# HansiZeng/scaling-retriever

Measured on AMD Instinct MI355X. Metric: MSMARCO-Dev queries/sec end-to-end (query encode + dense brute-force top-1000), higher is better.
Workload: dtype f32

## Files before the change

### include/sr_hip.h

```cpp
#ifndef SR_HIP_H
#define SR_HIP_H
#include <stdint.h>
#ifdef __cplusplus
extern "C" {
#endif

#define SR_OK 0
#define SR_ERR_INVALID 1
#define SR_ERR_HIP 2
#define SR_ERR_NOMEM 3
#define SR_ERR_UNSUPPORTED 4

#define SR_DTYPE_F32 0
#define SR_DTYPE_BF16 1
#define SR_DTYPE_F16 2

typedef void* sr_stream;

const char* sr_last_error(void);
int sr_version(void);
int sr_max_topk(void);

typedef struct sr_dense_index sr_dense_index;

// ... 250 lines not shown
                       const float* d_rope_cos, const float* d_rope_sin, int32_t n_rope, int32_t head_dim,
                       const float* d_bias, const int32_t* d_seq_of, const float* d_out_scale, int32_t out_nseg,
                       sr_stream stream);
int sr_gemm_qkv_rope(const void* d_A, const void* d_W, int32_t M, int32_t N, int32_t K, void* d_C,
                     const int32_t* d_pos, const float* d_rope_cos, const float* d_rope_sin,
                     int32_t n_rope, int32_t head_dim, sr_stream stream);
int sr_gemm_qkv_rope_bias(const void* d_A, const void* d_W, int32_t M, int32_t N, int32_t K, void* d_C,
                          const int32_t* d_pos, const float* d_rope_cos, const float* d_rope_sin,
                          int32_t n_rope, int32_t head_dim, const float* d_bias, int32_t fp32_out, sr_stream stream);
int sr_attention_varlen(const void* d_qkv, void* d_out, const int32_t* d_cu_seqlens, const int32_t* d_pos,
                        const uint8_t* d_key_valid, const float* d_rope_cos, const float* d_rope_sin,
                        int32_t B, int32_t num_heads, int32_t num_kv_heads, int32_t head_dim, sr_stream stream);
int sr_attention_varlen_f32(const float* d_qkv, float* d_out_f32, void* d_out_planes, int32_t fp32_planes,
                            const int32_t* d_cu_seqlens, const uint8_t* d_key_valid, int32_t B, int32_t num_heads,
                            int32_t num_kv_heads, int32_t head_dim, int32_t max_seqlen, sr_stream stream);
int sr_rmsnorm_bf16(float* d_x, const float* d_embed, const int32_t* d_tok_id, const void* d_delta, const float* d_norm_w,
                    void* d_xn, float* d_xn_f32, float eps, int32_t T, int32_t H, sr_stream stream);
int sr_dense_head_pool(const float* d_x, const float* d_norm_w, const int32_t* d_cu_seqlens, const int32_t* d_pos,
                       const int32_t* d_pool_start, float eps, int32_t B, int32_t T, int32_t H, void* d_stats, float* d_out,
                       sr_stream stream);
int sr_sparse_finish(float* d_out, int64_t n, float scale, int32_t round_bf16, sr_stream stream);
int sr_encode_plan(const int64_t* d_input_ids, const int64_t* d_attention_mask, int32_t B, int32_t L, int32_t mode, int32_t vocab,
                   const int32_t* d_row_shift, int32_t* d_span_start, int32_t* d_span_len, int32_t* d_pool_start,
                   int32_t* d_row_len, int32_t* d_cu_seqlens, int32_t* d_tok_id, int32_t* d_pos, uint8_t* d_key_valid,
                   int32_t* d_seq_of, int64_t capacity, int64_t* n_tokens, sr_stream stream);
int sr_split_bf16(const float* d_src, int64_t n, void* d_p0, void* d_p1, void* d_p2, sr_stream stream);
int sr_topk_replay(const float* d_scores, const int64_t* d_ids, int64_t nq, int64_t n_stream, const int64_t* h_steps, int n_steps,
                   int k, int k2, int64_t select_over, int filter, int seg_n, int seg_group, float tau2_init, float pad_score,
                   float* d_out_scores, int64_t* d_out_ids, int32_t* d_out_counts, float* d_trace_tau, float* d_trace_tau2,
                   int32_t* d_trace_cand, int32_t* d_trace_run, uint64_t* d_trace_keys, sr_stream stream);
// ... 22 lines not shown
```

### scaling_retriever_amd/_lib.py

```python
import contextlib
import ctypes
import os
import threading

_HERE = os.path.dirname(os.path.abspath(__file__))
LIB_PATH = os.environ.get("SR_HIP_LIB") or os.path.join(_HERE, "libsr_hip.so")

SR_OK, SR_ERR_INVALID, SR_ERR_HIP, SR_ERR_NOMEM, SR_ERR_UNSUPPORTED = 0, 1, 2, 3, 4
SR_DTYPE_F32, SR_DTYPE_BF16, SR_DTYPE_F16 = 0, 1, 2
SR_FUSE_RRF, SR_FUSE_MINMAX = 0, 1

c_void_p, c_int, c_int32, c_int64, c_float, c_char_p = (ctypes.c_void_p, ctypes.c_int, ctypes.c_int32,
                                                         ctypes.c_int64, ctypes.c_float, ctypes.c_char_p)


class SrModelConfig(ctypes.Structure):
    _fields_ = [
        ("vocab_size", c_int32), ("hidden_size", c_int32), ("intermediate_size", c_int32), ("num_layers", c_int32),
        ("num_heads", c_int32), ("num_kv_heads", c_int32), ("head_dim", c_int32),
        ("rms_norm_eps", c_float), ("rope_theta", c_float), ("rope_llama3", c_int32),
        ("rope_factor", c_float), ("rope_low_freq_factor", c_float), ("rope_high_freq_factor", c_float),
        ("rope_original_max_pos", c_int32), ("tie_word_embeddings", c_int32), ("has_lm_head", c_int32),
        ("max_batch_tokens", c_int32), ("max_batch_seqs", c_int32), ("fp32_planes", c_int32),
        ("attention_bias", c_int32),
# ... 135 lines not shown
    "sr_rmsnorm_bf16": (c_int, [c_void_p, c_void_p, c_void_p, c_void_p, c_void_p, c_void_p, c_void_p, c_float, c_int32, c_int32, c_void_p]),
    "sr_dense_head_pool": (c_int, [c_void_p, c_void_p, c_void_p, c_void_p, c_void_p, c_float, c_int32, c_int32, c_int32, c_void_p, c_void_p,
                                   c_void_p]),
    "sr_sparse_finish": (c_int, [c_void_p, c_int64, c_float, c_int32, c_void_p]),
    "sr_encode_plan": (c_int, [c_void_p, c_void_p, c_int32, c_int32, c_int32, c_int32, c_void_p, c_void_p, c_void_p, c_void_p, c_void_p,
                               c_void_p, c_void_p, c_void_p, c_void_p, c_void_p, c_int64, ctypes.POINTER(c_int64), c_void_p]),
    "sr_split_bf16": (c_int, [c_void_p, c_int64, c_void_p, c_void_p, c_void_p, c_void_p]),
    "sr_gemm_qkv_rope": (c_int, [c_void_p, c_void_p, c_int32, c_int32, c_int32, c_void_p, c_void_p, c_void_p, c_void_p,
                                 c_int32, c_int32, c_void_p]),
    "sr_gemm_qkv_rope_bias": (c_int, [c_void_p, c_void_p, c_int32, c_int32, c_int32, c_void_p, c_void_p, c_void_p, c_void_p,
                                      c_int32, c_int32, c_void_p, c_int32, c_void_p]),
    "sr_attention_varlen": (c_int, [c_void_p, c_void_p, c_void_p, c_void_p, c_void_p, c_void_p, c_void_p, c_int32,
                                    c_int32, c_int32, c_int32, c_void_p]),
    "sr_attention_varlen_f32": (c_int, [c_void_p, c_void_p, c_void_p, c_int32, c_void_p, c_void_p, c_int32, c_int32, c_int32,
                                        c_int32, c_int32, c_void_p]),
    "sr_sparse_compact": (c_int, [c_void_p, c_int64, c_int64, c_void_p, c_void_p, c_void_p, c_int64,
                                  ctypes.POINTER(c_int64), c_void_p]),
    "sr_sparse_compact_topm": (c_int, [c_void_p, c_int64, c_int64, c_int64, c_void_p, c_void_p, c_void_p, c_int64,
                                       ctypes.POINTER(c_int64), c_void_p]),
}

_lib = None
_lock = threading.Lock()


class SrHipError(RuntimeError):
    pass


def _bind(path):
    if not os.path.exists(path):
        raise SrHipError(
            f"{path} not found: the HIP extension is not built. There is no CPU fallback; "
            "run `make -C scaling_retriever_amd/csrc` (needs hipcc, targets gfx950).")
    import torch
    lib = ctypes.CDLL(path)
    for name, (res, args) in SIGNATURES.items():
        fn = getattr(lib, name)
        fn.restype = res
        fn.argtypes = args
    return lib


def load():
    global _lib
    with _lock:
        if _lib is None:
            _lib = _bind(LIB_PATH)
        return _lib


@contextlib.contextmanager
def library(path):
    global _lib
    other = _bind(os.path.abspath(path))
    with _lock:
        keep, _lib = _lib, other
    try:
        yield other
    finally:
        with _lock:
            _lib = keep


def check(rc, what=""):
    if rc == SR_OK:
        return
    msg = load().sr_last_error().decode("utf-8", "replace")
    if rc == SR_ERR_INVALID:
        raise ValueError(f"{what}: {msg}" if what else msg)
# ... 16 lines not shown
```

### scaling_retriever_amd/csrc/api.hip

```cpp
#include "kernels.h"
#include <stdlib.h>
#include <string>
#include <vector>

static thread_local std::string g_last_error;

void sr_set_error(const char* fmt, ...) {
    char buf[1024];
    va_list ap;
    va_start(ap, fmt);
    vsnprintf(buf, sizeof(buf), fmt, ap);
    va_end(ap);
    g_last_error = buf;
}

int sr_cu_count() {
    static int per_dev[SR_MAX_DEVICES] = {};
    int d = 0;
    if (hipGetDevice(&d) != hipSuccess || d < 0 || d >= SR_MAX_DEVICES) d = 0;
    if (per_dev[d] == 0) {
        int n = 0;
        if (hipDeviceGetAttribute(&n, hipDeviceAttributeMultiprocessorCount, d) != hipSuccess || n <= 0) { (void)hipGetLastError(); n = 256; }
        per_dev[d] = n;
    }
// ... 65 lines not shown
extern "C" int sr_attention_varlen_f32(const float* d_qkv, float* d_out_f32, void* d_out_planes, int32_t fp32_planes,
                                       const int32_t* d_cu_seqlens, const uint8_t* d_key_valid, int32_t B, int32_t num_heads,
                                       int32_t num_kv_heads, int32_t head_dim, int32_t max_seqlen, sr_stream stream) {
    SR_REQUIRE(d_qkv && d_cu_seqlens && d_key_valid, "sr_attention_varlen_f32: null pointer");
    SR_REQUIRE((d_out_f32 != nullptr) != (d_out_planes != nullptr), "sr_attention_varlen_f32: pass exactly one of d_out_f32 / d_out_planes");
    SR_REQUIRE(d_out_f32 || fp32_planes == 2 || fp32_planes == 3, "sr_attention_varlen_f32: fp32_planes %d (2 or 3 for plane output)", fp32_planes);
    SR_REQUIRE(B >= 0 && max_seqlen >= 0 && num_heads > 0 && num_kv_heads > 0 && head_dim > 0, "sr_attention_varlen_f32: bad sizes");
    SR_REQUIRE((uintptr_t)d_qkv % 16 == 0 && (uintptr_t)d_out_f32 % 16 == 0 && (uintptr_t)d_out_planes % 8 == 0,
               "sr_attention_varlen_f32: d_qkv and d_out_f32 must be 16-byte aligned, d_out_planes 8-byte aligned");
    AttnF32Args a{};
    a.qkv = d_qkv; a.out_f32 = d_out_f32; a.out = (bf16_t*)d_out_planes; a.cu_seqlens = d_cu_seqlens; a.key_valid = d_key_valid;
    a.B = B; a.nh = num_heads; a.nkv = num_kv_heads; a.hd = head_dim;
    a.scale = 1.0f / sqrtf((float)head_dim); a.max_seqlen = max_seqlen;
    if (!d_out_f32) a.out_map = split_map_a(fp32_planes);
    return launch_attention_f32(a, (hipStream_t)stream);
}

extern "C" int sr_gemm_f16_scaled(const void* d_A, const void* d_W, int32_t M, int32_t N, int32_t K, const float* d_a_scale,
                                  const float* d_w_scale, float* d_C, sr_stream stream) {
    SR_REQUIRE(d_A && d_W && d_C && d_a_scale && d_w_scale, "sr_gemm_f16_scaled: null pointer");
    GemmArgs g{};
    g.A = (const bf16_t*)d_A; g.W = (const bf16_t*)d_W; g.M = M; g.N = N; g.K = K; g.C = d_C; g.a_scale = d_a_scale; g.w_scale = d_w_scale;
    return launch_gemm_bf16(EPI_RESID_F32_H, g, (hipStream_t)stream);
}

extern "C" int sr_rows_split_f16(float* d_src, const float* d_embed, const int32_t* d_tok_id, const float* d_norm_w, float eps,
                                 int32_t T, int32_t K, int32_t nseg, void* d_planes, float* d_a_inv, const float* d_gu_cmax,
                                 float* d_act_sc, float* d_act_inv, sr_stream stream) {
    SR_REQUIRE(d_src && d_planes && d_a_inv, "sr_rows_split_f16: null pointer");
    SR_REQUIRE((d_embed == nullptr) == (d_tok_id == nullptr), "sr_rows_split_f16: pass both d_embed and d_tok_id or neither");
// ... 103 lines not shown
```

### scaling_retriever_amd/csrc/attention_f32.hip

```cpp
#include "kernels.h"
#include <math.h>

#define AF_KC 64
#define AF_RPW 4
#define AF_ROWS 16

__device__ inline float af_mul_rn(float a, float b) {
#pragma clang fp contract(off)
    return a * b;
}

template <int HD>
__global__ __launch_bounds__(256) void attention_f32_kernel(AttnF32Args a) {
    constexpr int DPL = HD / 64;
    __shared__ float Ks[AF_KC][HD + 1];
    __shared__ float qs[AF_ROWS][HD];
    __shared__ float ps[AF_ROWS][AF_KC];
    __shared__ unsigned char kval[AF_KC];
    const int b = blockIdx.x, h = blockIdx.y;
    const int tid = threadIdx.x, lane = tid & 63, wave = tid >> 6;
    const int t0 = a.cu_seqlens[b];
    const int S = a.cu_seqlens[b + 1] - t0;
    const int r0 = blockIdx.z * AF_ROWS;
    if (r0 >= S || S <= a.only_gt) return;
// ... 210 lines not shown
    const float s0 = af_quad_xor(hi1 ? x0 : x1, 0xB1), s1 = af_quad_xor(hi1 ? x2 : x3, 0xB1);
    if (hi1) { x0 = s0; x2 = s1; } else { x1 = s0; x3 = s1; }
    x = f32x4{x0, x1, x2, x3};
}

__host__ __device__ constexpr int af_mfma_waves(int hd, int nkb) {
    return nkb == 0 ? 1 : (hd == 64 ? (nkb == 1 ? 8 : 6) : (nkb <= 2 ? 5 : 4));
}

template <int HD, int NKB>
__global__ __launch_bounds__(256, af_mfma_waves(HD, NKB)) void attention_f32_mfma_kernel(AttnF32Args a) {
    constexpr int LDK = HD + 1, CB = HD / 16;
    constexpr bool OLD = NKB == 0;
    constexpr int MKB = OLD ? 4 : NKB;
    extern __shared__ float af_smem[];
    const int b = blockIdx.x, kvh = blockIdx.y;
    const int tid = threadIdx.x, lane = tid & 63, wave = tid >> 6;
    const int t0 = a.cu_seqlens[b];
    const int S = a.cu_seqlens[b + 1] - t0;
    if (S <= 0 || S > a.only_le) return;
    const int nkb = (S + 15) >> 4;
    if (!OLD && (a.nkb_only ? nkb != a.nkb_only : nkb > NKB)) return;
    const int SP = nkb * 16;
    float* Ks = af_smem;
    float* Vs = Ks + SP * LDK;
    const int G = a.nh / a.nkv;
    const int h = kvh * G + wave;
    const int ld = (a.nh + 2 * a.nkv) * HD;
    const int koff = a.nh * HD + kvh * HD, voff = (a.nh + a.nkv) * HD + kvh * HD;
    const int g = lane >> 4, c = lane & 15;
    f32x4 qv[CB];
    auto load_q = [&](int qb) {
#pragma unroll
        for (int i = 0; i < CB; ++i) {
// ... 161 lines not shown
                    bf16_t* orow = a.out + (int64_t)(t0 + row) * ldo;
                    for (int sg = 0; sg < a.out_map.n_seg; ++sg) {
                        const int pl = a.out_map.plane[sg];
                        bf16x4 w;
#pragma unroll
                        for (int e = 0; e < 4; ++e) w[e] = (short)(pl == 0 ? p[e][0] : (pl == 1 ? p[e][1] : p[e][2]));
                        *reinterpret_cast<bf16x4*>(orow + (int64_t)sg * a.nh * HD + col) = w;
                    }
                }
            }
        }
    }
}

template <int HD, int NKB>
static int launch_attention_f32_mfma_cfg(const AttnF32Args& a, size_t lds, hipStream_t s) {
    static DeviceOnce attr_once;
    if (bool* slot = attr_once.pending()) {
        constexpr int max_sp = NKB ? 16 * NKB : 64;
        SR_CHECK_HIP(hipFuncSetAttribute(reinterpret_cast<const void*>(&attention_f32_mfma_kernel<HD, NKB>),
                                         hipFuncAttributeMaxDynamicSharedMemorySize, (int)(sizeof(float) * (2 * max_sp + (NKB ? 0 : 64)) * (HD + 1))));
        *slot = true;
    }
    const dim3 grid((unsigned)a.B, (unsigned)a.nkv), block(256);
    SR_REQUIRE(grid.y <= 65535, "attention(fp32): grid too large");
    hipLaunchKernelGGL((attention_f32_mfma_kernel<HD, NKB>), grid, block, lds, s, a);
    SR_CHECK_LAUNCH();
    return SR_OK;
}

template <int HD>
static int launch_attention_f32_mfma_class(const AttnF32Args& a, int nkb, hipStream_t s) {
    const size_t lds = sizeof(float) * (size_t)(2 * 16 * nkb) * (HD + 1);
    switch (nkb) {
        case 1: return launch_attention_f32_mfma_cfg<HD, 1>(a, lds, s);
        case 2: return launch_attention_f32_mfma_cfg<HD, 2>(a, lds, s);
        case 3: return launch_attention_f32_mfma_cfg<HD, 3>(a, lds, s);
        default: return launch_attention_f32_mfma_cfg<HD, 4>(a, lds, s);
    }
}

template <int HD>
static int launch_attention_f32_mfma(const AttnF32Args& a_in, hipStream_t s) {
    AttnF32Args a = a_in;
    const int top = (int)ceil_div64(a.max_seqlen < 64 ? a.max_seqlen : 64, 16);
    const char* env = sr_dev_getenv("SR_ATTN_F32_LAYOUT");
    if (env && *env == '0') {
        const size_t lds = sizeof(float) * (size_t)(2 * 16 * top + 4 * 16) * (HD + 1);
        return launch_attention_f32_mfma_cfg<HD, 0>(a, lds, s);
    }
    const bool force = env && *env == '2';
    if (!a.have_classes && !force) {
        a.nkb_only = 0;
        return launch_attention_f32_mfma_class<HD>(a, top, s);
    }
    for (int nkb = 1; nkb <= top; ++nkb) {
        if (a.have_classes && a.class_seqs[nkb - 1] == 0) continue;
        a.nkb_only = nkb;
        SR_TRY(launch_attention_f32_mfma_class<HD>(a, nkb, s));
    }
    return SR_OK;
}

int launch_attention_f32(const AttnF32Args& a_in, hipStream_t s) {
    AttnF32Args a = a_in;
    SR_REQUIRE(a.nh % a.nkv == 0, "attention(fp32): num_heads %d not a multiple of num_kv_heads %d", a.nh, a.nkv);
    SR_REQUIRE(a.out_f32 || (a.out_map.n_seg >= 1 && a.out_map.n_seg <= SR_MAX_SEG), "attention(fp32): bad segment map");
    if (a.B == 0 || a.max_seqlen <= 0) return SR_OK;
    const int G = a.nh / a.nkv;
    a.only_le = 0; a.only_gt = 0;
    const char* env_m = sr_dev_getenv("SR_ATTN_F32_MFMA");
    if (G == 4 && (a.hd == 64 || a.hd == 128) && !(env_m && *env_m == '0')) {
        a.only_le = 64;
        SR_TRY(a.hd == 64 ? launch_attention_f32_mfma<64>(a, s) : launch_attention_f32_mfma<128>(a, s));
// ... 26 lines not shown
```

### scaling_retriever_amd/csrc/encoder.hip

```cpp
#include "encoder_model.h"
#include <math.h>

struct Pass {
    sr_model* m;
    hipStream_t s;
    int B, T;
    int max_len;
    int attn_class[4];
    bool fused_on, fused_all;
};

static int ensure_fp32_workspace(sr_model* m) {
    if (m->xs) return SR_OK;
    const sr_model_config& c = m->cfg;
    SR_REQUIRE(c.fp32_planes > 0, "encode(fp32): the model was created with fp32_planes = 0 (bf16 regime only)");
    const int64_t Tm = m->Tm, nsg = split_map_a(c.fp32_planes).n_seg;
    const ModelDims& d = m->d;
    DeviceArena& mem = m->mem_fp32;
    auto allocate = [&]() -> int {
        SR_TRY(mem.alloc(m->xs, Tm * d.H * nsg, true));
        SR_TRY(mem.alloc(m->qkv_f, Tm * d.n_qkv, true));
        SR_TRY(mem.alloc(m->attn_s, Tm * d.nq * nsg, true));
        SR_TRY(mem.alloc(m->act_s, Tm * d.I * nsg, true));
        if (c.fp32_planes != SR_FP32_PLANES_F16) return SR_OK;
        SR_TRY(mem.alloc(m->attn_f, Tm * d.nq, true));
        SR_TRY(mem.alloc(m->act_f, Tm * d.I, true));
        SR_TRY(mem.alloc(m->xs_i, Tm, true));
        SR_TRY(mem.alloc(m->attn_i, Tm, true));
        SR_TRY(mem.alloc(m->act_i, Tm, true));
        SR_TRY(mem.alloc(m->act_sc, Tm, true));
        return SR_OK;
    };
    if (allocate() != SR_OK) {
        mem.release();
        sr_set_error("encode(fp32): hipMalloc of the fp32-regime workspace failed (%lld tokens)", (long long)Tm);
        return SR_ERR_NOMEM;
    }
    return SR_OK;
// ... 9 lines not shown
    g.a_nseg = nseg; g.a_scale = a_inv; g.w_scale = w_inv;
    return g;
}
static void set_rope(GemmArgs& g, const sr_model* m, const float* bias) {
    g.pos = m->pos; g.rope_cos = m->rope_cos; g.rope_sin = m->rope_sin; g.n_rope = m->d.nq + m->d.nkv; g.head_dim = m->d.hd;
    g.bias = bias;
}
static AttnF32Args attn_f32_args(const Pass& p) {
    const sr_model* m = p.m;
    AttnF32Args a{};
    a.qkv = m->qkv_f; a.cu_seqlens = m->cu; a.key_valid = m->key_valid;
    a.B = p.B; a.nh = m->cfg.num_heads; a.nkv = m->cfg.num_kv_heads; a.hd = m->d.hd;
    a.scale = 1.0f / sqrtf((float)m->d.hd); a.max_seqlen = p.max_len;
    a.have_classes = 1;
    for (int n = 0; n < 4; ++n) a.class_seqs[n] = p.attn_class[n];
    return a;
}
static int split_rows(const Pass& p, float* src, const float* w, bf16_t* dst, float* inv, int K, int nseg) {
    return launch_rows_split_f16(src, nullptr, nullptr, w, dst, inv, p.T, K, p.m->cfg.rms_norm_eps, nseg, nullptr, nullptr, nullptr, p.s);
}

static int layer_bf16(const Pass& p, int li) {
    sr_model* m = p.m;
    const ModelDims& d = m->d;
    const LayerW& l = m->layers[li];
    const float eps = m->cfg.rms_norm_eps;
    const int T = p.T;
    hipStream_t s = p.s;
    if (li == 0) SR_TRY(launch_rmsnorm(m->x, m->embed, m->tok_id, nullptr, l.ln1, m->xn, nullptr, T, d.H, eps, s));
    else SR_TRY(launch_rmsnorm(m->x, nullptr, nullptr, m->delta, l.ln1, m->xn, nullptr, T, d.H, eps, s));
// ... 54 lines not shown
    SR_TRY(launch_gemm_bf16(EPI_RESID_F32_H, gemm_f16(m->attn_s, m->attn_i, l.wo_s, l.wo_i, l.o_seg, T, d.H, d.nq, m->x), s));
    if (p.fused_on && (l.fused_act || p.fused_all)) {
        SR_TRY(launch_rows_split_f16(m->x, nullptr, nullptr, l.ln2, m->xs, m->xs_i, T, d.H, eps, l.gu_seg, m->gu_cmax + li, m->act_sc,
                                     m->act_i, s));
        g = gemm_f16(m->xs, m->xs_i, l.wgu_s, l.wgu_i, l.gu_seg, T, 2 * d.I, d.H, m->act_s);
        g.out_scale = m->act_sc; g.out_nseg = l.down_seg;
        SR_TRY(launch_gemm_bf16(EPI_SWIGLU_SPLIT_H, g, s));
    } else {
        SR_TRY(split_rows(p, m->x, l.ln2, m->xs, m->xs_i, d.H, l.gu_seg));
        SR_TRY(launch_gemm_bf16(EPI_SWIGLU_F32_H, gemm_f16(m->xs, m->xs_i, l.wgu_s, l.wgu_i, l.gu_seg, T, 2 * d.I, d.H, m->act_f), s));
        SR_TRY(split_rows(p, m->act_f, nullptr, m->act_s, m->act_i, d.I, l.down_seg));
    }
    return launch_gemm_bf16(EPI_RESID_F32_H, gemm_f16(m->act_s, m->act_i, l.wdown_s, l.wdown_i, l.down_seg, T, d.H, d.I, m->x), s);
}

static int plan_batch(sr_model* m, const int64_t* d_ids, const int64_t* d_mask, int B, int L, int mode, const int32_t* d_shift, Pass& p) {
    hipStream_t s = p.s;
    SR_TRY(launch_plan_rows(d_mask, B, L, mode, m->span_start, m->span_len, m->pool_start, m->row_len, d_shift, m->cu, s));
    SR_CHECK_HIP(hipMemcpyAsync(m->h_cu, m->cu, (size_t)(B + 1) * 4, hipMemcpyDeviceToHost, s));
    SR_CHECK_HIP(hipStreamSynchronize(s));
    p.B = B;
    p.T = m->h_cu[B];
    p.max_len = 0;
    for (int n = 0; n < 4; ++n) p.attn_class[n] = 0;
    for (int b = 0; b < B; ++b) {
        const int len = m->h_cu[b + 1] - m->h_cu[b];
        p.max_len = len > p.max_len ? len : p.max_len;
        if (len >= 1 && len <= 64) ++p.attn_class[(len - 1) >> 4];
    }
    SR_REQUIRE(p.T <= m->Tm, "encode: batch packs to %d tokens, workspace holds %d (raise max_batch_tokens or split the batch)", p.T, m->Tm);
    m->last_T = p.T;
    if (p.T == 0) return SR_OK;
    return launch_plan_tokens(d_ids, d_mask, B, L, m->span_start, m->cu, m->tok_id, m->pos, m->key_valid, m->seq_of, m->d.V, mode, d_shift, s);
}

static int model_forward(sr_model* m, const int64_t* d_ids, const int64_t* d_mask, int B, int L, int mode, int prec, const int32_t* d_shift,
                         Pass& p) {
    const sr_model_config& c = m->cfg;
    SR_REQUIRE(m->finalized, "encode: sr_model_finalize was not called");
    SR_REQUIRE(B >= 1 && L >= 1, "encode: bad batch shape [%d, %d]", B, L);
    SR_REQUIRE(B <= m->Bm, "encode: batch of %d sequences exceeds max_batch_seqs %d", B, m->Bm);
    SR_REQUIRE(L <= m->max_pos, "encode: sequence length %d exceeds %d", L, m->max_pos);
    SR_REQUIRE(d_ids && d_mask, "encode: null input");
    if (prec == PREC_FP32) SR_TRY(ensure_fp32_workspace(m));
    SR_TRY(plan_batch(m, d_ids, d_mask, B, L, mode, d_shift, p));
    if (p.T == 0) return SR_OK;
    const bool f16p = prec == PREC_FP32 && c.fp32_planes == SR_FP32_PLANES_F16;
    if (f16p) {
        const char* env_fa = sr_dev_getenv("SR_FP32_FUSED_ACT");
        p.fused_on = !(env_fa && *env_fa == '0');
        p.fused_all = env_fa && *env_fa == '1';
    }
    for (int li = 0; li < c.num_layers; ++li)
        SR_TRY(prec == PREC_BF16 ? layer_bf16(p, li) : (f16p ? layer_f16_planes(p, li) : layer_f32_planes(p, li)));
    if (prec == PREC_BF16)
        SR_TRY(launch_rmsnorm(m->x, nullptr, nullptr, m->delta, nullptr, nullptr, nullptr, p.T, m->d.H, c.rms_norm_eps, p.s));
    return SR_OK;
}

static int head_dense(const Pass& p, int prec, float* d_out) {
// ... 108 lines not shown
```

### scaling_retriever_amd/csrc/encoder_kernels.hip

```cpp
#include "kernels.h"
#include <math.h>

__global__ void plan_rows_kernel(const int64_t* __restrict__ mask, int B, int L, int mode, int* __restrict__ span_start,
                                 int* __restrict__ span_len, int* __restrict__ pool_start, int* __restrict__ row_len,
                                 const int* __restrict__ row_shift) {
    const int b = blockIdx.x;
    const int lane = threadIdx.x;
    int len = 0, first = L, last = -1;
    for (int p = lane; p < L; p += 64) {
        if (mask[(int64_t)b * L + p] != 0) {
            ++len;
            first = p < first ? p : first;
            last = p > last ? p : last;
        }
    }
    for (int off = 32; off > 0; off >>= 1) {
        len += __shfl_xor(len, off);
        const int f = __shfl_xor(first, off), l = __shfl_xor(last, off);
        first = f < first ? f : first;
        last = l > last ? l : last;
    }
    if (lane == 0) {
        int st, ln, ps;
        if (len == 0) {
// ... 19 lines not shown
    const int tid = threadIdx.x;
    const int per = (B + 255) / 256;
    const int b0 = tid * per, b1 = (b0 + per) < B ? (b0 + per) : B;
    int s = 0;
    for (int b = b0; b < b1; ++b) s += span_len[b];
    part[tid] = s;
    __syncthreads();
    if (tid == 0) {
        int run = 0;
        for (int i = 0; i < 256; ++i) { const int v = part[i]; part[i] = run; run += v; }
        cu[B] = run;
    }
    __syncthreads();
    int run = part[tid];
    for (int b = b0; b < b1; ++b) { cu[b] = run; run += span_len[b]; }
}

__global__ void plan_tokens_kernel(const int64_t* __restrict__ ids, const int64_t* __restrict__ mask, int L,
                                   const int* __restrict__ span_start, const int* __restrict__ cu, int* __restrict__ tok_id,
                                   int* __restrict__ pos, unsigned char* __restrict__ key_valid, int* __restrict__ seq_of,
                                   int vocab, int mode, const int* __restrict__ row_shift) {
    const int b = blockIdx.x;
    const int t0 = cu[b], n = cu[b + 1] - t0, st = span_start[b];
    const int shift = row_shift ? row_shift[b] : 0;
    for (int j = threadIdx.x; j < n; j += blockDim.x) {
        const int p = st + j;
        int64_t id = ids[(int64_t)b * L + p];
        id = id < 0 ? 0 : (id >= vocab ? vocab - 1 : id);
        tok_id[t0 + j] = (int)id;
        pos[t0 + j] = p - shift < 0 ? 0 : p - shift;
        const bool valid = mask[(int64_t)b * L + p] != 0;
        key_valid[t0 + j] = valid ? 1 : 0;
        seq_of[t0 + j] = (mode != 0 && !valid) ? -2 : b;
    }
}

int launch_plan_rows(const int64_t* mask, int B, int L, int mode, int* span_start, int* span_len, int* pool_start, int* row_len,
                     const int* row_shift, int* cu, hipStream_t s) {
    hipLaunchKernelGGL(plan_rows_kernel, dim3(B), dim3(64), 0, s, mask, B, L, mode, span_start, span_len, pool_start, row_len, row_shift);
    hipLaunchKernelGGL(plan_scan_kernel, dim3(1), dim3(256), 0, s, span_len, B, cu);
    SR_CHECK_LAUNCH();
    return SR_OK;
}
int launch_plan_tokens(const int64_t* ids, const int64_t* mask, int B, int L, const int* span_start, const int* cu, int* tok_id, int* pos,
                       unsigned char* key_valid, int* seq_of, int vocab, int mode, const int* row_shift, hipStream_t s) {
    hipLaunchKernelGGL(plan_tokens_kernel, dim3(B), dim3(128), 0, s, ids, mask, L, span_start, cu, tok_id, pos, key_valid, seq_of, vocab,
                       mode, row_shift);
    SR_CHECK_LAUNCH();
    return SR_OK;
}

template <int NCH>
__global__ __launch_bounds__(256) void rmsnorm_kernel(float* __restrict__ x, const float* __restrict__ embed,
                                                      const int* __restrict__ tok_id, const bf16_t* __restrict__ delta,
                                                      const float* __restrict__ w, bf16_t* __restrict__ xn,
                                                      float* __restrict__ xn_f32, int T, int H, float eps) {
    const int t = blockIdx.x * 4 + (threadIdx.x >> 6);
    const int lane = threadIdx.x & 63;
// ... 200 lines not shown
```

### scaling_retriever_amd/csrc/encoder_model.h

```cpp
#pragma once
#include "kernels.h"
#include <mutex>
#include <vector>

enum { PREC_BF16 = 0, PREC_FP32 = 1 };

struct ModelDims {
    int H, I, V;
    int nq, nkv;
    int n_qkv;
    int hd;
};

struct DeviceArena {
    struct Block { void* p; void** slot; };
    std::vector<Block> blocks;
    DeviceArena() = default;
    DeviceArena(const DeviceArena&) = delete;
    DeviceArena& operator=(const DeviceArena&) = delete;
    ~DeviceArena() { release(); }
    template <typename T>
    int alloc(T*& ptr, int64_t n, bool zero = false) {
        const size_t bytes = (size_t)n * sizeof(T);
        void* p = nullptr;
// ... 55 lines not shown
    bf16_t* xn = nullptr;
    bf16_t* qkv = nullptr;
    bf16_t* attn = nullptr;
    bf16_t* act = nullptr;
    bf16_t* delta = nullptr;
    int *span_start = nullptr, *span_len = nullptr, *pool_start = nullptr, *row_len = nullptr, *cu = nullptr;
    int *tok_id = nullptr, *pos = nullptr, *seq_of = nullptr;
    unsigned char* key_valid = nullptr;
    bf16_t* xs = nullptr;
    float* qkv_f = nullptr;
    bf16_t* attn_s = nullptr;
    bf16_t* act_s = nullptr;
    float *attn_f = nullptr, *act_f = nullptr;
    float *xs_i = nullptr, *attn_i = nullptr, *act_i = nullptr;
    float* act_sc = nullptr;
    DeviceArena mem;
    DeviceArena mem_fp32;
    int* h_cu = nullptr;
    int last_T = 0;
    std::mutex mu;
    StreamOrder order;

    sr_model() = default;
    sr_model(const sr_model&) = delete;
    ~sr_model() {
        if (h_cu) (void)hipHostFree(h_cu);
        order.release();
    }
};
```

### scaling_retriever_amd/csrc/gemm_bf16.hip

```cpp
#include "kernels.h"
#include <math.h>
#include <stdlib.h>
#include <string.h>
#include <type_traits>

typedef __bf16 mfma_bf16x8 __attribute__((ext_vector_type(8)));
typedef _Float16 mfma_f16x8 __attribute__((ext_vector_type(8)));
template <bool F16>
__device__ __forceinline__ f32x4 sr_mma(const mfma_bf16x8& w, const mfma_bf16x8& a, const f32x4& c) {
    if constexpr (F16)
        return __builtin_amdgcn_mfma_f32_16x16x32_f16(__builtin_bit_cast(mfma_f16x8, w), __builtin_bit_cast(mfma_f16x8, a), c, 0, 0, 0);
    else
        return __builtin_amdgcn_mfma_f32_16x16x32_bf16(w, a, c, 0, 0, 0);
}
__device__ __forceinline__ f32x4 sr_rope_lo(const f32x4& x1, const f32x4& x2, const f32x4& c, const f32x4& s) {
#pragma clang fp contract(off)
    f32x4 y;
#pragma unroll
    for (int r = 0; r < 4; ++r) { const float a = x1[r] * c[r], b = x2[r] * s[r]; y[r] = a - b; }
    return y;
}
__device__ __forceinline__ f32x4 sr_rope_hi(const f32x4& x1, const f32x4& x2, const f32x4& c, const f32x4& s) {
#pragma clang fp contract(off)
    f32x4 y;
// ... 672 lines not shown
                const int tok = it * 4 + (lane_e >> 4), pl = (lane_e >> 3) & 1, pc = lane_e & 7;
                const sr_i32x4 v = *reinterpret_cast<const sr_i32x4*>(stg + tok * 256 + pl * 128 + ((pc ^ (tok & 7)) << 4));
                const int m = mrow + tok, n = nb + pc * 8;
                if (m < g.M && n < half_n) {
                    bf16_t* crow = out_c + (int64_t)m * ldc + n;
                    if (pl == 0) {
                        *reinterpret_cast<sr_i32x4*>(crow) = v;
                    } else {
                        *reinterpret_cast<sr_i32x4*>(crow + half_n) = v;
                        if (seg3) *reinterpret_cast<sr_i32x4*>(crow + 2 * half_n) = v;
                    }
                }
            }
            __builtin_amdgcn_sched_barrier(0);
        }
    } else if constexpr (BEPI == EPI_STORE_BF16 || BEPI == EPI_STORE_F32 || BEPI == EPI_RESID_F32) {
#pragma unroll
        for (int j = 0; j < MB; ++j) {
            const int m = m0 + wm * MB * 16 + j * 16 + frow;
            if (m >= g.M) continue;
#pragma unroll
            for (int i = 0; i < NB; ++i) {
                const int n = n0 + wn * NB * 16 + i * 16 + fg * 4;
                if (n >= g.N) continue;
                const f32x4 v = acc[i][j];
                if constexpr (BEPI == EPI_STORE_BF16) {
                    bf16x4 o;
                    o[0] = (short)f32_to_bf16(v[0]);
                    o[1] = (short)f32_to_bf16(v[1]);
                    o[2] = (short)f32_to_bf16(v[2]);
                    o[3] = (short)f32_to_bf16(v[3]);
                    *reinterpret_cast<bf16x4*>(reinterpret_cast<bf16_t*>(g.C) + (int64_t)m * g.N + n) = o;
                } else if constexpr (BEPI == EPI_STORE_F32) {
                    *reinterpret_cast<f32x4*>(reinterpret_cast<float*>(g.C) + (int64_t)m * g.N + n) = v;
                } else {
                    f32x4* p = reinterpret_cast<f32x4*>(reinterpret_cast<float*>(g.C) + (int64_t)m * g.N + n);
                    f32x4 x = *p;
                    x += v;
                    *p = x;
                }
            }
        }
    } else if constexpr (E::QKV_ROPE) {
        constexpr bool F32OUT = E::OUT_BYTES == 4;
        const int hd = g.head_dim, hb = hd / 32;
        auto put = [&](int64_t off, const f32x4& v) {
            if constexpr (F32OUT) {
                *reinterpret_cast<f32x4*>(reinterpret_cast<float*>(g.C) + off) = v;
            } else {
                bf16x4 o;
#pragma unroll
                for (int r = 0; r < 4; ++r) o[r] = (short)f32_to_bf16(v[r]);
                *reinterpret_cast<bf16x4*>(reinterpret_cast<bf16_t*>(g.C) + off) = o;
            }
// ... 366 lines not shown
```

### scaling_retriever_amd/csrc/kernels.h

```cpp
#pragma once
#include "common.h"

typedef unsigned short bf16_t;

enum GemmEpilogue {
    EPI_STORE_BF16 = 0,
    EPI_RESID_F32 = 1,
    EPI_SWIGLU = 2,
    EPI_SEGMAX = 3,
    EPI_STORE_F32 = 4,
    EPI_QKV_ROPE = 5,
    EPI_QKV_ROPE_F32 = 6,
    EPI_SWIGLU_SPLIT = 7,
    EPI_SWIGLU_F32 = 8,
    EPI_H_FIRST = 9,
    EPI_QKV_ROPE_F32_H = 9, EPI_RESID_F32_H = 10, EPI_SWIGLU_F32_H = 11, EPI_SEGMAX_H = 12,
    EPI_SWIGLU_SPLIT_H = 13,
    EPI_SWIGLU_SPLITH_BASE = 14,
};

#define SR_MAX_SEG 6
struct SplitMap {
    int n_seg;
    int plane[SR_MAX_SEG];
// ... 35 lines not shown
int launch_gemm_bf16(GemmEpilogue epi, const GemmArgs& g, hipStream_t s);

int launch_rows_split_f16(float* x, const float* embed, const int* tok, const float* w, bf16_t* xs, float* inv, int T, int K, float eps,
                          int nseg, const float* gu_cmax, float* act_sc, float* act_inv, hipStream_t s);
int launch_gu_cmax(const bf16_t* wgu_s, const float* wgu_i, int I, int K, int nseg, float* cmax, hipStream_t s);
int launch_gu_pair_samples(const bf16_t* wgu_s, const float* wgu_i, int I, int K, int nseg, int ns, float* p, hipStream_t s);

int launch_rmsnorm_split(float* x, const float* embed, const int* tok_id, const float* w, bf16_t* xs, int T, int H, float eps,
                         const SplitMap& map, hipStream_t s);
int launch_rmsnorm(float* x, const float* embed, const int* tok_id, const bf16_t* delta, const float* w, bf16_t* xn, float* xn_f32, int T,
                   int H, float eps, hipStream_t s);
int launch_plan_rows(const int64_t* mask, int B, int L, int mode, int* span_start, int* span_len, int* pool_start, int* row_len,
                     const int* row_shift, int* cu, hipStream_t s);
int launch_plan_tokens(const int64_t* ids, const int64_t* mask, int B, int L, const int* span_start, const int* cu, int* tok_id, int* pos,
                       unsigned char* key_valid, int* seq_of, int vocab, int mode, const int* row_shift, hipStream_t s);
int launch_dense_head(const float* x, const float* w, float2* stats, const int* cu, const int* pos, const int* pool_start, float* out,
                      int B, int T, int H, float eps, hipStream_t s);
int launch_sparse_finish(float* out, int64_t n, float scale, int round_bf16, hipStream_t s);

struct AttnArgs {
    const bf16_t* qkv;
    bf16_t* out;
    const int* cu_seqlens;
    const int* pos;
    const unsigned char* key_valid;
    const float* rope_cos;
    const float* rope_sin;
    int B, nh, nkv, hd;
    float scale;
    int apply_rope;
// ... 2 lines not shown
int launch_attention(const AttnArgs& a, hipStream_t s);

struct AttnF32Args {
    const float* qkv;
    float* out_f32;
    bf16_t* out;
    const int* cu_seqlens;
    const unsigned char* key_valid;
    int B, nh, nkv, hd;
    float scale;
    int max_seqlen;
    SplitMap out_map;
    int only_le = 0, only_gt = 0;
    int have_classes = 0, class_seqs[4] = {0, 0, 0, 0};
    int nkb_only = 0;
};
int launch_attention_f32(const AttnF32Args& a, hipStream_t s);
```

Before: 16000.

## Compact attention grids per length class and batch residual epilogue loads

Adds a device planning kernel that buckets sequences by key-block count (length classes up to 64) and writes compact (start,len) spans, so each per-class fp32 attention launch covers only its own sequences instead of launching B blocks that mostly exit early. The GEMM residual epilogue is split out so it loads all residual fragments for a row before adding and storing, which aims to overlap memory latency. It also adds a public API entry for class-based attention and lets the Python binding tolerate missing symbols. The cost is an extra small single-block kernel during planning.

Measured after the change: 16000 (median of 3 runs). No clear change (+0.0%).

```diff
diff --git a/include/sr_hip.h b/include/sr_hip.h
--- a/include/sr_hip.h
+++ b/include/sr_hip.h
@@ -288,6 +288,9 @@
 int sr_attention_varlen_f32(const float* d_qkv, float* d_out_f32, void* d_out_planes, int32_t fp32_planes,
                             const int32_t* d_cu_seqlens, const uint8_t* d_key_valid, int32_t B, int32_t num_heads,
                             int32_t num_kv_heads, int32_t head_dim, int32_t max_seqlen, sr_stream stream);
+int sr_attention_varlen_f32_classes(const float* d_qkv, float* d_out_f32, void* d_out_planes, int32_t fp32_planes,
+                                    const int32_t* d_cu_seqlens, const uint8_t* d_key_valid, int32_t B, int32_t num_heads,
+                                    int32_t num_kv_heads, int32_t head_dim, int32_t* d_class_spans, sr_stream stream);
 int sr_rmsnorm_bf16(float* d_x, const float* d_embed, const int32_t* d_tok_id, const void* d_delta, const float* d_norm_w,
                     void* d_xn, float* d_xn_f32, float eps, int32_t T, int32_t H, sr_stream stream);
 int sr_dense_head_pool(const float* d_x, const float* d_norm_w, const int32_t* d_cu_seqlens, const int32_t* d_pos,
diff --git a/scaling_retriever_amd/_lib.py b/scaling_retriever_amd/_lib.py
--- a/scaling_retriever_amd/_lib.py
+++ b/scaling_retriever_amd/_lib.py
@@ -173,6 +173,8 @@
                                     c_int32, c_int32, c_int32, c_void_p]),
     "sr_attention_varlen_f32": (c_int, [c_void_p, c_void_p, c_void_p, c_int32, c_void_p, c_void_p, c_int32, c_int32, c_int32,
                                         c_int32, c_int32, c_void_p]),
+    "sr_attention_varlen_f32_classes": (c_int, [c_void_p, c_void_p, c_void_p, c_int32, c_void_p, c_void_p, c_int32, c_int32, c_int32,
+                                                c_int32, c_void_p, c_void_p]),
     "sr_sparse_compact": (c_int, [c_void_p, c_int64, c_int64, c_void_p, c_void_p, c_void_p, c_int64,
                                   ctypes.POINTER(c_int64), c_void_p]),
     "sr_sparse_compact_topm": (c_int, [c_void_p, c_int64, c_int64, c_int64, c_void_p, c_void_p, c_void_p, c_int64,
@@ -187,7 +189,7 @@
     pass
 
 
-def _bind(path):
+def _bind(path, allow_missing=False):
     if not os.path.exists(path):
         raise SrHipError(
             f"{path} not found: the HIP extension is not built. There is no CPU fallback; "
@@ -195,6 +197,8 @@
     import torch
     lib = ctypes.CDLL(path)
     for name, (res, args) in SIGNATURES.items():
+        if allow_missing and not hasattr(lib, name):
+            continue
         fn = getattr(lib, name)
         fn.restype = res
         fn.argtypes = args
@@ -205,14 +209,14 @@
     global _lib
     with _lock:
         if _lib is None:
-            _lib = _bind(LIB_PATH)
+            _lib = _bind(LIB_PATH, allow_missing=bool(os.environ.get("SR_HIP_LIB")))
         return _lib
 
 
 @contextlib.contextmanager
 def library(path):
     global _lib
-    other = _bind(os.path.abspath(path))
+    other = _bind(os.path.abspath(path), allow_missing=True)
     with _lock:
         keep, _lib = _lib, other
     try:
diff --git a/scaling_retriever_amd/csrc/api.hip b/scaling_retriever_amd/csrc/api.hip
--- a/scaling_retriever_amd/csrc/api.hip
+++ b/scaling_retriever_amd/csrc/api.hip
@@ -103,6 +103,36 @@
     a.scale = 1.0f / sqrtf((float)head_dim); a.max_seqlen = max_seqlen;
     if (!d_out_f32) a.out_map = split_map_a(fp32_planes);
     return launch_attention_f32(a, (hipStream_t)stream);
+}
+
+extern "C" int sr_attention_varlen_f32_classes(const float* d_qkv, float* d_out_f32, void* d_out_planes, int32_t fp32_planes,
+                                               const int32_t* d_cu_seqlens, const uint8_t* d_key_valid, int32_t B, int32_t num_heads,
+                                               int32_t num_kv_heads, int32_t head_dim, int32_t* d_class_spans, sr_stream stream) {
+    SR_REQUIRE(d_qkv && d_cu_seqlens && d_key_valid && d_class_spans, "sr_attention_varlen_f32_classes: null pointer");
+    SR_REQUIRE((d_out_f32 != nullptr) != (d_out_planes != nullptr), "sr_attention_varlen_f32_classes: pass exactly one of d_out_f32 / d_out_planes");
+    SR_REQUIRE(d_out_f32 || fp32_planes == 2 || fp32_planes == 3, "sr_attention_varlen_f32_classes: fp32_planes %d (2 or 3 for plane output)", fp32_planes);
+    SR_REQUIRE(B >= 0 && B <= 65536 && num_heads > 0 && num_kv_heads > 0 && head_dim > 0, "sr_attention_varlen_f32_classes: bad sizes");
+    SR_REQUIRE((uintptr_t)d_qkv % 16 == 0 && (uintptr_t)d_out_f32 % 16 == 0 && (uintptr_t)d_out_planes % 8 == 0 && (uintptr_t)d_class_spans % 8 == 0,
+               "sr_attention_varlen_f32_classes: d_qkv and d_out_f32 must be 16-byte aligned, d_out_planes and d_class_spans 8-byte aligned");
+    if (B == 0) return SR_OK;
+    hipStream_t s = (hipStream_t)stream;
+    AttnF32Args a{};
+    a.qkv = d_qkv; a.out_f32 = d_out_f32; a.out = (bf16_t*)d_out_planes; a.cu_seqlens = d_cu_seqlens; a.key_valid = d_key_valid;
+    a.B = B; a.nh = num_heads; a.nkv = num_kv_heads; a.hd = head_dim;
+    a.scale = 1.0f / sqrtf((float)head_dim);
+    if (!d_out_f32) a.out_map = split_map_a(fp32_planes);
+    SR_TRY(launch_plan_classes(d_cu_seqlens, B, reinterpret_cast<int2*>(d_class_spans), s));
+    std::vector<int> cu((size_t)B + 1);
+    SR_CHECK_HIP(hipMemcpyAsync(cu.data(), d_cu_seqlens, sizeof(int) * ((size_t)B + 1), hipMemcpyDeviceToHost, s));
+    SR_CHECK_HIP(hipStreamSynchronize(s));
+    a.have_classes = 1;
+    a.class_spans = reinterpret_cast<const int2*>(d_class_spans);
+    for (int b = 0; b < B; ++b) {
+        const int len = cu[b + 1] - cu[b];
+        a.max_seqlen = len > a.max_seqlen ? len : a.max_seqlen;
+        if (len >= 1 && len <= 64) ++a.class_seqs[(len - 1) >> 4];
+    }
+    return launch_attention_f32(a, s);
 }
 
 extern "C" int sr_gemm_f16_scaled(const void* d_A, const void* d_W, int32_t M, int32_t N, int32_t K, const float* d_a_scale,
diff --git a/scaling_retriever_amd/csrc/attention_f32.hip b/scaling_retriever_amd/csrc/attention_f32.hip
--- a/scaling_retriever_amd/csrc/attention_f32.hip
+++ b/scaling_retriever_amd/csrc/attention_f32.hip
@@ -248,10 +248,17 @@
     constexpr bool OLD = NKB == 0;
     constexpr int MKB = OLD ? 4 : NKB;
     extern __shared__ float af_smem[];
-    const int b = blockIdx.x, kvh = blockIdx.y;
+    const int kvh = blockIdx.y;
     const int tid = threadIdx.x, lane = tid & 63, wave = tid >> 6;
-    const int t0 = a.cu_seqlens[b];
-    const int S = a.cu_seqlens[b + 1] - t0;
+    int t0, S;
+    if (a.seq_spans) {
+        const int2 sp = a.seq_spans[blockIdx.x];
+        t0 = sp.x;
+        S = sp.y;
+    } else {
+        t0 = a.cu_seqlens[blockIdx.x];
+        S = a.cu_seqlens[blockIdx.x + 1] - t0;
+    }
     if (S <= 0 || S > a.only_le) return;
     const int nkb = (S + 15) >> 4;
     if (!OLD && (a.nkb_only ? nkb != a.nkb_only : nkb > NKB)) return;
@@ -443,7 +450,7 @@
 }
 
 template <int HD, int NKB>
-static int launch_attention_f32_mfma_cfg(const AttnF32Args& a, size_t lds, hipStream_t s) {
+static int launch_attention_f32_mfma_cfg(const AttnF32Args& a, int n_seqs, size_t lds, hipStream_t s) {
     static DeviceOnce attr_once;
     if (bool* slot = attr_once.pending()) {
         constexpr int max_sp = NKB ? 16 * NKB : 64;
@@ -451,7 +458,7 @@
                                          hipFuncAttributeMaxDynamicSharedMemorySize, (int)(sizeof(float) * (2 * max_sp + (NKB ? 0 : 64)) * (HD + 1))));
         *slot = true;
     }
-    const dim3 grid((unsigned)a.B, (unsigned)a.nkv), block(256);
+    const dim3 grid((unsigned)n_seqs, (unsigned)a.nkv), block(256);
     SR_REQUIRE(grid.y <= 65535, "attention(fp32): grid too large");
     hipLaunchKernelGGL((attention_f32_mfma_kernel<HD, NKB>), grid, block, lds, s, a);
     SR_CHECK_LAUNCH();
@@ -459,34 +466,41 @@
 }
 
 template <int HD>
-static int launch_attention_f32_mfma_class(const AttnF32Args& a, int nkb, hipStream_t s) {
+static int launch_attention_f32_mfma_class(const AttnF32Args& a, int nkb, int n_seqs, hipStream_t s) {
     const size_t lds = sizeof(float) * (size_t)(2 * 16 * nkb) * (HD + 1);
     switch (nkb) {
-        case 1: return launch_attention_f32_mfma_cfg<HD, 1>(a, lds, s);
-        case 2: return launch_attention_f32_mfma_cfg<HD, 2>(a, lds, s);
-        case 3: return launch_attention_f32_mfma_cfg<HD, 3>(a, lds, s);
-        default: return launch_attention_f32_mfma_cfg<HD, 4>(a, lds, s);
+        case 1: return launch_attention_f32_mfma_cfg<HD, 1>(a, n_seqs, lds, s);
+        case 2: return launch_attention_f32_mfma_cfg<HD, 2>(a, n_seqs, lds, s);
+        case 3: return launch_attention_f32_mfma_cfg<HD, 3>(a, n_seqs, lds, s);
+        default: return launch_attention_f32_mfma_cfg<HD, 4>(a, n_seqs, lds, s);
     }
 }
 
 template <int HD>
 static int launch_attention_f32_mfma(const AttnF32Args& a_in, hipStream_t s) {
     AttnF32Args a = a_in;
+    a.seq_spans = nullptr;
     const int top = (int)ceil_div64(a.max_seqlen < 64 ? a.max_seqlen : 64, 16);
     const char* env = sr_dev_getenv("SR_ATTN_F32_LAYOUT");
     if (env && *env == '0') {
         const size_t lds = sizeof(float) * (size_t)(2 * 16 * top + 4 * 16) * (HD + 1);
-        return launch_attention_f32_mfma_cfg<HD, 0>(a, lds, s);
+        return launch_attention_f32_mfma_cfg<HD, 0>(a, a.B, lds, s);
     }
     const bool force = env && *env == '2';
     if (!a.have_classes && !force) {
         a.nkb_only = 0;
-        return launch_attention_f32_mfma_class<HD>(a, top, s);
-    }
+        return launch_attention_f32_mfma_class<HD>(a, top, a.B, s);
+    }
+    const bool listed = a.have_classes && a.class_spans != nullptr;
+    int first = 0;
     for (int nkb = 1; nkb <= top; ++nkb) {
-        if (a.have_classes && a.class_seqs[nkb - 1] == 0) continue;
+        const int n = a.have_classes ? a.class_seqs[nkb - 1] : 0;
+        if (a.have_classes && n == 0) continue;
+        SR_REQUIRE(n >= 0 && first + n <= a.B, "attention(fp32): class counts exceed the batch of %d sequences", a.B);
         a.nkb_only = nkb;
-        SR_TRY(launch_attention_f32_mfma_class<HD>(a, nkb, s));
+        a.seq_spans = listed ? a.class_spans + first : nullptr;
+        SR_TRY(launch_attention_f32_mfma_class<HD>(a, nkb, listed ? n : a.B, s));
+        first += n;
     }
     return SR_OK;
 }
diff --git a/scaling_retriever_amd/csrc/encoder.hip b/scaling_retriever_amd/csrc/encoder.hip
--- a/scaling_retriever_amd/csrc/encoder.hip
+++ b/scaling_retriever_amd/csrc/encoder.hip
@@ -22,6 +22,7 @@
         SR_TRY(mem.alloc(m->qkv_f, Tm * d.n_qkv, true));
         SR_TRY(mem.alloc(m->attn_s, Tm * d.nq * nsg, true));
         SR_TRY(mem.alloc(m->act_s, Tm * d.I * nsg, true));
+        SR_TRY(mem.alloc(m->attn_spans, m->Bm));
         if (c.fp32_planes != SR_FP32_PLANES_F16) return SR_OK;
         SR_TRY(mem.alloc(m->attn_f, Tm * d.nq, true));
         SR_TRY(mem.alloc(m->act_f, Tm * d.I, true));
@@ -61,6 +62,7 @@
     a.scale = 1.0f / sqrtf((float)m->d.hd); a.max_seqlen = p.max_len;
     a.have_classes = 1;
     for (int n = 0; n < 4; ++n) a.class_seqs[n] = p.attn_class[n];
+    a.class_spans = m->attn_spans;
     return a;
 }
 static int split_rows(const Pass& p, float* src, const float* w, bf16_t* dst, float* inv, int K, int nseg) {
@@ -145,9 +147,11 @@
     return launch_gemm_bf16(EPI_RESID_F32_H, gemm_f16(m->act_s, m->act_i, l.wdown_s, l.wdown_i, l.down_seg, T, d.H, d.I, m->x), s);
 }
 
-static int plan_batch(sr_model* m, const int64_t* d_ids, const int64_t* d_mask, int B, int L, int mode, const int32_t* d_shift, Pass& p) {
+static int plan_batch(sr_model* m, const int64_t* d_ids, const int64_t* d_mask, int B, int L, int mode, int prec, const int32_t* d_shift,
+                      Pass& p) {
     hipStream_t s = p.s;
     SR_TRY(launch_plan_rows(d_mask, B, L, mode, m->span_start, m->span_len, m->pool_start, m->row_len, d_shift, m->cu, s));
+    if (prec == PREC_FP32) SR_TRY(launch_plan_classes(m->cu, B, m->attn_spans, s));
     SR_CHECK_HIP(hipMemcpyAsync(m->h_cu, m->cu, (size_t)(B + 1) * 4, hipMemcpyDeviceToHost, s));
     SR_CHECK_HIP(hipStreamSynchronize(s));
     p.B = B;
@@ -174,7 +178,7 @@
     SR_REQUIRE(L <= m->max_pos, "encode: sequence length %d exceeds %d", L, m->max_pos);
     SR_REQUIRE(d_ids && d_mask, "encode: null input");
     if (prec == PREC_FP32) SR_TRY(ensure_fp32_workspace(m));
-    SR_TRY(plan_batch(m, d_ids, d_mask, B, L, mode, d_shift, p));
+    SR_TRY(plan_batch(m, d_ids, d_mask, B, L, mode, prec, d_shift, p));
     if (p.T == 0) return SR_OK;
     const bool f16p = prec == PREC_FP32 && c.fp32_planes == SR_FP32_PLANES_F16;
     if (f16p) {
diff --git a/scaling_retriever_amd/csrc/encoder_kernels.hip b/scaling_retriever_amd/csrc/encoder_kernels.hip
--- a/scaling_retriever_amd/csrc/encoder_kernels.hip
+++ b/scaling_retriever_amd/csrc/encoder_kernels.hip
@@ -57,6 +57,38 @@
     __syncthreads();
     int run = part[tid];
     for (int b = b0; b < b1; ++b) { cu[b] = run; run += span_len[b]; }
+}
+
+__global__ void plan_classes_kernel(const int* __restrict__ cu, int B, int2* __restrict__ spans) {
+    __shared__ int cnt[4][256];
+    __shared__ int total[4];
+    const int tid = threadIdx.x;
+    const int per = (B + 255) / 256;
+    const int b0 = tid * per, b1 = (b0 + per) < B ? (b0 + per) : B;
+    int c[4] = {0, 0, 0, 0};
+    for (int b = b0; b < b1; ++b) {
+        const int len = cu[b + 1] - cu[b];
+        if (len >= 1 && len <= 64) ++c[(len - 1) >> 4];
+    }
+#pragma unroll
+    for (int n = 0; n < 4; ++n) cnt[n][tid] = c[n];
+    __syncthreads();
+    if (tid < 4) {
+        int run = 0;
+        for (int i = 0; i < 256; ++i) { const int v = cnt[tid][i]; cnt[tid][i] = run; run += v; }
+        total[tid] = run;
+    }
+    __syncthreads();
+    int at[4], first = 0;
+#pragma unroll
+    for (int n = 0; n < 4; ++n) { at[n] = first + cnt[n][tid]; first += total[n]; }
+    for (int b = b0; b < b1; ++b) {
+        const int t0 = cu[b], len = cu[b + 1] - t0;
+        if (len < 1 || len > 64) continue;
+        const int n = (len - 1) >> 4;
+        const int o = n == 0 ? at[0]++ : (n == 1 ? at[1]++ : (n == 2 ? at[2]++ : at[3]++));
+        spans[o] = make_int2(t0, len);
+    }
 }
 
 __global__ void plan_tokens_kernel(const int64_t* __restrict__ ids, const int64_t* __restrict__ mask, int L,
@@ -85,6 +117,11 @@
     SR_CHECK_LAUNCH();
     return SR_OK;
 }
+int launch_plan_classes(const int* cu, int B, int2* spans, hipStream_t s) {
+    hipLaunchKernelGGL(plan_classes_kernel, dim3(1), dim3(256), 0, s, cu, B, spans);
+    SR_CHECK_LAUNCH();
+    return SR_OK;
+}
 int launch_plan_tokens(const int64_t* ids, const int64_t* mask, int B, int L, const int* span_start, const int* cu, int* tok_id, int* pos,
                        unsigned char* key_valid, int* seq_of, int vocab, int mode, const int* row_shift, hipStream_t s) {
     hipLaunchKernelGGL(plan_tokens_kernel, dim3(B), dim3(128), 0, s, ids, mask, L, span_start, cu, tok_id, pos, key_valid, seq_of, vocab,
diff --git a/scaling_retriever_amd/csrc/encoder_model.h b/scaling_retriever_amd/csrc/encoder_model.h
--- a/scaling_retriever_amd/csrc/encoder_model.h
+++ b/scaling_retriever_amd/csrc/encoder_model.h
@@ -93,6 +93,7 @@
     float *attn_f = nullptr, *act_f = nullptr;
     float *xs_i = nullptr, *attn_i = nullptr, *act_i = nullptr;
     float* act_sc = nullptr;
+    int2* attn_spans = nullptr;
     DeviceArena mem;
     DeviceArena mem_fp32;
     int* h_cu = nullptr;
diff --git a/scaling_retriever_amd/csrc/gemm_bf16.hip b/scaling_retriever_amd/csrc/gemm_bf16.hip
--- a/scaling_retriever_amd/csrc/gemm_bf16.hip
+++ b/scaling_retriever_amd/csrc/gemm_bf16.hip
@@ -710,7 +710,30 @@
             }
             __builtin_amdgcn_sched_barrier(0);
         }
-    } else if constexpr (BEPI == EPI_STORE_BF16 || BEPI == EPI_STORE_F32 || BEPI == EPI_RESID_F32) {
+    } else if constexpr (BEPI == EPI_RESID_F32) {
+        float* const cf = reinterpret_cast<float*>(g.C);
+#pragma unroll
+        for (int j = 0; j < MB; ++j) {
+            const int m = m0 + wm * MB * 16 + j * 16 + frow;
+            const float* row = cf + (int64_t)(m < g.M ? m : g.M - 1) * g.N;
+            f32x4 x[NB];
+#pragma unroll
+            for (int i = 0; i < NB; ++i) {
+                const int n = n0 + wn * NB * 16 + i * 16 + fg * 4;
+                x[i] = *reinterpret_cast<const f32x4*>(row + (n < g.N ? n : g.N - 4));
+            }
+            __builtin_amdgcn_sched_barrier(0);
+#pragma unroll
+            for (int i = 0; i < NB; ++i) {
+                const int n = n0 + wn * NB * 16 + i * 16 + fg * 4;
+                if (m >= g.M || n >= g.N) continue;
+                f32x4 y = x[i];
+                y += acc[i][j];
+                *reinterpret_cast<f32x4*>(cf + (int64_t)m * g.N + n) = y;
+            }
+            __builtin_amdgcn_sched_barrier(0);
+        }
+    } else if constexpr (BEPI == EPI_STORE_BF16 || BEPI == EPI_STORE_F32) {
 #pragma unroll
         for (int j = 0; j < MB; ++j) {
             const int m = m0 + wm * MB * 16 + j * 16 + frow;
@@ -727,13 +750,8 @@
                     o[2] = (short)f32_to_bf16(v[2]);
                     o[3] = (short)f32_to_bf16(v[3]);
                     *reinterpret_cast<bf16x4*>(reinterpret_cast<bf16_t*>(g.C) + (int64_t)m * g.N + n) = o;
-                } else if constexpr (BEPI == EPI_STORE_F32) {
+                } else {
                     *reinterpret_cast<f32x4*>(reinterpret_cast<float*>(g.C) + (int64_t)m * g.N + n) = v;
-                } else {
-                    f32x4* p = reinterpret_cast<f32x4*>(reinterpret_cast<float*>(g.C) + (int64_t)m * g.N + n);
-                    f32x4 x = *p;
-                    x += v;
-                    *p = x;
                 }
             }
         }
diff --git a/scaling_retriever_amd/csrc/kernels.h b/scaling_retriever_amd/csrc/kernels.h
--- a/scaling_retriever_amd/csrc/kernels.h
+++ b/scaling_retriever_amd/csrc/kernels.h
@@ -73,6 +73,7 @@
                      const int* row_shift, int* cu, hipStream_t s);
 int launch_plan_tokens(const int64_t* ids, const int64_t* mask, int B, int L, const int* span_start, const int* cu, int* tok_id, int* pos,
                        unsigned char* key_valid, int* seq_of, int vocab, int mode, const int* row_shift, hipStream_t s);
+int launch_plan_classes(const int* cu, int B, int2* spans, hipStream_t s);
 int launch_dense_head(const float* x, const float* w, float2* stats, const int* cu, const int* pos, const int* pool_start, float* out,
                       int B, int T, int H, float eps, hipStream_t s);
 int launch_sparse_finish(float* out, int64_t n, float scale, int round_bf16, hipStream_t s);
@@ -105,5 +106,7 @@
     int only_le = 0, only_gt = 0;
     int have_classes = 0, class_seqs[4] = {0, 0, 0, 0};
     int nkb_only = 0;
+    const int2* class_spans = nullptr;
+    const int2* seq_spans = nullptr;
 };
 int launch_attention_f32(const AttnF32Args& a, hipStream_t s);
```
